# calad0i/da4ml

Hardware: AMD Instinct MI355X
Metric: CMVM solves/sec, 256x256 int8 matrix (higher is better)
Workload: dtype u32; 1 GPU; c3_256x256_int8_batch64_single_chain; matrix=256x256 int8 (default_rng(seed).integers(-128,128)), batch_per_gpu=64, parallelism=1 x independent-instance shard, no data-path collective

## Files before the change

da4ml_amd/csrc/cmvm_engine.hip:

```cpp

#include <hip/hip_runtime.h>

#include <algorithm>
#include <atomic>
#include <chrono>
#include <cmath>
#include <cstdio>
#include <cstdlib>
#include <cstring>
#include <memory>
#include <mutex>
#include <numeric>
#include <stdexcept>
#include <string>
#include <thread>
#include <type_traits>
#include <vector>

#include "cmvm_core.h"
#include "cmvm_geometry.h"
#include "cmvm_gpu.h"
#include "cmvm_host.h"

namespace da {
// ... 1383 lines not shown
            if constexpr (MANYCOL) {
                if (!same) rlB[pos - 1] = F::pack(colA, nbv);
            } else {
                if (!same) s_bent[pos - 1] = F::pack(colA, nbv);
            }
            rlN[at] = F::pack(colA, ma);
            mcol[at] = (int)colA;
            mA[at] = ma;
            mB[at] = mb;
            s_cm[colA] = (Idx)(at + 1);
            {
                DA_GLOBAL uint32_t *cb = colbits + (size_t)colA * cbw;
                atomicOr(gen(&cb[Nw >> 5]), 1u << (Nw & 31));
                if (na == 0) atomicAnd(gen(&cb[A >> 5]), ~(1u << (A & 31)));
                if (!same && nbv == 0) atomicAnd(gen(&cb[B >> 5]), ~(1u << (B & 31)));
            }
            if constexpr (MANYCOL)
                s_len[at] = collen[colA];
            else
                s_len[at] = s_clen[colA];
            s_col[at] = (Idx)colA;
            my_matches += popc32(O::plus(ma) | O::minus(ma));
        }
        if (na) for_pairs_self<Cell>(na, nb, [&](int k) { atomicAdd(&cAA[k], 1u); });
        if (!same) {
            if (na && nbv) for_pairs_cross<Cell>(na, nbv, nb, [&](int k) { atomicAdd(&cAB[k], 1u); });
            if (nbv && ma) for_pairs_cross<Cell>(nbv, ma, nb, [&](int k) { atomicAdd(&cBN[k], 1u); });
        }
        if (na && ma) for_pairs_cross<Cell>(na, ma, nb, [&](int k) { atomicAdd(&cAN[k], 1u); });
        if (ma) for_pairs_self<Cell>(ma, nb, [&](int k) { atomicAdd(&cNN[k], 1u); });
        m += chunk;
        __syncthreads();
    }
    if (my_matches) atomicAdd(&s_matches, my_matches);
    if (!same)
        for (int t = tid; t < lenB; t += SEL2_THREADS) {
            Entry e;
            if constexpr (MANYCOL)
                e = rlB[t];
            else {
                e = s_bent[t];
                rlB[t] = e;
            }
            const Cell nbv = F::cell(e);
            if (nbv) for_pairs_self<Cell>(nbv, nb, [&](int k) { atomicAdd(&cBB[k], 1u); });
        }
    for (int j = tid; j < n_out; j += SEL2_THREADS) cmap[j] = (uint16_t)s_cm[j];
    {
        const unsigned long long refN = ref_pack(Nw, (uint32_t)m, offN);
        for (int k = tid; k < m; k += SEL2_THREADS) {
            const int j = s_col[k], len = s_len[k];
            if (len < lcap) {
                collist[(size_t)j * lcap + len] = refN;
                collen[j] = len + 1;
            } else
                g->error = E_LIST_CAPACITY;
        }
    }
    __syncthreads();
    SEL_TIMER_MARK(4)
    SEL_TIMER_MARK(5)
    if constexpr (SHARDED) {
        for (int k = tid; k < 6 * c.K; k += SEL2_THREADS) {
            const int sp = k / c.K;
            cs_slab[k] = (same && (sp == 1 || sp == 2 || sp == 4)) ? 0 : (int32_t)s_cnt[sp * Kpad + (k - sp * c.K)];
        }
    } else
        for (int k = tid; k < 6 * Kpad; k += SEL2_THREADS) sp_cnt[k] = s_cnt[k];
    {
        const DA_GLOBAL uint32_t *cb = colbits;
        const int nwords = (int)((Nw + 31) >> 5), chunks = (nwords + WAVE - 1) / WAVE;
        DA_GLOBAL uint32_t *ids = pl_ids;
        const bool split = chunks * 4 <= NW && m >= 8 && nwords <= claim_words;
        if (split) {
            const int c = wid % chunks, part = wid / chunks, ways = (NW - c + chunks - 1) / chunks;
            const int w = c * WAVE + lane;
            if (w < nwords) {
                uint32_t bits = 0;
                for (int k = part; k < m; k += ways) bits |= cb[(size_t)s_col[k] * cbw + w];
                if (bits) atomicOr(&s_or[w], bits);
            }
            __syncthreads();
        }
        for (int wb = wid * WAVE; wb < nwords; wb += SEL2_THREADS) {
            const int w = wb + lane;
            uint32_t bits = 0;
            if (w < nwords) {
                if (split)
                    bits = s_or[w];
                else
                    for (int k = 0; k < m; ++k) bits |= cb[(size_t)s_col[k] * cbw + w];
                if ((int)(A >> 5) == w) bits &= ~(1u << (A & 31));
                if ((int)(B >> 5) == w) bits &= ~(1u << (B & 31));
                if ((int)(Nw >> 5) == w) bits &= ~(1u << (Nw & 31));
            }
            if constexpr (SHARDED) {
                const int fw = (int)((Nw + 3) / 4);
                if (w < nwords) {
#pragma unroll
                    for (int q = 0; q < 8; ++q) {
                        const uint32_t b = (bits >> (4 * q)) & 0xFu;
                        if (8 * w + q < fw) cs_flags[8 * w + q] = (int32_t)((b & 1u) | ((b & 2u) << 7) | ((b & 4u) << 14) | ((b & 8u) << 21));
                    }
                }
                continue;
            }
            const int cnt = popc32(bits), inc = (int)wave_scan_add_u32((uint32_t)cnt);
            const int wave_total = __builtin_amdgcn_readlane(inc, WAVE - 1);
            if (wave_total == 0) continue;
            int base = 0;
            if (lane == 0) base = atomicAdd(&s_np, wave_total);
            int at = __builtin_amdgcn_readfirstlane(base) + inc - cnt;
            while (bits) {
                const uint32_t id = (uint32_t)(w << 5) + (uint32_t)ctz32(bits);
                if (at < IDS_LDS)
                    s_ids[at] = id;
                else
                    ids[at] = id;
                ++at;
                bits &= bits - 1;
            }
        }
    }
    SEL_TIMER_MARK(6)
    __syncthreads();
    if constexpr (SHARDED) {
        if (tid < SHARD_TRAILER) cs_flags[(int)((Nw + 3) / 4) + tid] = 0;
    }
    {
        const int np = s_np;
        const DA_GLOBAL uint32_t *ids = pl_ids;
        for (int t = tid; t < np; t += 2 * SEL2_THREADS) {
            const int t2 = t + SEL2_THREADS;
            const bool has2 = t2 < np;
            const uint32_t r1 = t < IDS_LDS ? s_ids[t] : ids[t];
            const uint32_t r2 = !has2 ? r1 : t2 < IDS_LDS ? s_ids[t2] : ids[t2];
            const da_u2 ro1 = rowoff[r1], ro2 = rowoff[r2];
            load_fence();
            plist[t] = ref_pack(r1, ro1.y, ro1.x);
            if (has2) plist[t2] = ref_pack(r2, ro2.y, ro2.x);
        }
    }
    SEL_TIMER_MARK(7)
    if (tid == 0) {
        SEL_TIMER_FLUSH
        rowoff[Nw] = da_u2{offN, (uint32_t)m};
        g->rl_used = offN + (uint32_t)m;
        g->m = m;
        g->n_partners = s_np;
        atomicAdd(&g->st_matches, (unsigned long long)s_matches);
        atomicAdd(&g->st_partners, (unsigned long long)s_np);
        atomicAdd(&g->st_cells, (unsigned long long)s_np * (unsigned)m);
        if (fast) atomicAdd(&g->st_fast, 1ull);
        {
            const unsigned long long eb = sizeof(Entry), cb = sizeof(Cell);
            const unsigned long long nwords = (Nw + 31) >> 5;
            atomicAdd(&g->st_sel_bytes, 4ull * (unsigned)n_out + 64ull + 2ull * eb * (unsigned)(lenA + (same ? 0 : lenB)) + 4ull * (unsigned)m * nwords + 20ull * (unsigned)s_np +
                                            (unsigned)m * (4ull + 2ull * cb + eb + 8ull + 12ull) + 2ull * (unsigned)n_out + 6ull * 4ull * (unsigned)Kpad);
        }
        g->A = A;
        g->B = B;
        g->Nw = Nw;
        g->pk_shift = shift;
        g->pk_sub = sub;
        g->n_rows = (int)Nw + 1;
        g->iter = iter + 1;
    }
    return 0;
}
#ifndef DA_SEL2_WAVES
#define DA_SEL2_WAVES 4
#endif
template <class Cell, bool SHARDED = false, bool MANYCOL = false, bool SEEDED = false> __global__ void __launch_bounds__(SEL2_THREADS) __attribute__((amdgpu_waves_per_eu(DA_SEL2_WAVES, DA_SEL2_WAVES))) k_iter_select2(ChainDev *chains, int n_chains, unsigned int *n_done, int step) {
    if ((int)blockIdx.x >= n_chains) return;
#ifdef DA_STEP_CLOCKS
    {
        ChainDev *g = &chains[blockIdx.x];
        if (threadIdx.x == 0 && !g->done) {
            CLK_MARK(g, step & 1, 0, true);
            if (blockIdx.y == 1 && step > 0) {
                unsigned long long *k = g->clk[(step - 1) & 1];
                if (k[0] && k[1] && k[2] && k[3] && CLK_TIMED_STEP(step - 1)) {
                    g->st_qdiag[0] += k[1] - ~k[0];
                    g->st_qdiag[1] += ~k[2] - k[1];
                    g->st_qdiag[4] += k[3] - ~k[2];
                    g->st_qdiag[5] += CLK_NOW() - k[3];
                    g->st_qdiag[7] += 1;
                }
                k[0] = k[1] = k[2] = k[3] = 0;
            }
        }
    }
#endif
    if (blockIdx.y == 0)
        search_body<Cell, SEEDED>(&chains[blockIdx.x], step);
    else
        (void)pick_body<Cell, SHARDED, MANYCOL, SEEDED>(&chains[blockIdx.x], n_done, step);
#ifdef DA_STEP_CLOCKS
    __syncthreads();
    if (threadIdx.x == 0) CLK_MARK(&chains[blockIdx.x], step & 1, 1, false);
#endif
}

#ifndef DA_UPD_OCC
#define DA_UPD_OCC 5
#endif
#if DA_UPD_OCC >= 8
#define DA_UPD_SGPRS 80
#elif DA_UPD_OCC == 7
#define DA_UPD_SGPRS 96
#else
#define DA_UPD_SGPRS 102
#endif
constexpr int SLOT_NONE = -1, SLOT_SLOW = -2;

#ifndef DA_UPD_QG
#define DA_UPD_QG 16
#endif
constexpr int QG = DA_UPD_QG, QN = WAVE / QG;
constexpr int QG_LOG2 = QG == 16 ? 4 : 3, SPL = (int)BUCKET / QG, HL = QG / 2;
constexpr uint32_t QMASK = (1u << QG) - 1u, HMASK = (1u << HL) - 1u;
static_assert(QG == 16 || QG == 8, "a partner row is handled by one DPP row or half a row");

__device__ __forceinline__ unsigned long long row_max_u64(unsigned long long v) {
    v = dpp_max_u64<DPP_ROW_SHR1, 0xF>(v);
    v = dpp_max_u64<DPP_ROW_SHR2, 0xF>(v);
    v = dpp_max_u64<DPP_ROW_SHR4, 0xF>(v);
    v = dpp_max_u64<DPP_ROW_SHR8, 0xF>(v);
    return v;
}

constexpr int DPP_QUAD_XOR1 = 0xB1, DPP_QUAD_XOR2 = 0x4E, DPP_ROW_HALF_MIRROR = 0x141;
template <int LANES> __device__ __forceinline__ unsigned long long part_row_max_u64(unsigned long long v) {
    v = dpp_max_u64<DPP_QUAD_XOR1, 0xF>(v);
    v = dpp_max_u64<DPP_QUAD_XOR2, 0xF>(v);
    if constexpr (LANES == 8) v = dpp_max_u64<DPP_ROW_HALF_MIRROR, 0xF>(v);
    return v;
}

template <class Cell> struct UpdStep {
    Ctx c;
    int done, n_partners, m, n_in;
    uint32_t A, B, Nw;
    int shift, sub;
    const DA_GLOBAL int *mcol;
    const DA_GLOBAL Cell *mA, *mB;
    const DA_GLOBAL uint16_t *cmap;
    const DA_GLOBAL typename RowFmt<Cell>::Entry *rl;
    const DA_GLOBAL unsigned long long *plist;
    uint32_t dcw;
};
template <class Cell, bool SEEDED = false, bool WEIGHTED = false> __device__ __forceinline__ UpdStep<Cell> load_upd_step(ChainDev *gq) {
    using Entry = typename RowFmt<Cell>::Entry;
    UpdStep<Cell> u;
    int iter = gq->iter;
    u.done = gq->done, u.n_partners = gq->n_partners, u.m = gq->m, u.n_in = gq->n_in;
    u.A = gq->A, u.B = gq->B, u.Nw = gq->Nw;
    u.shift = gq->pk_shift, u.sub = gq->pk_sub;
    u.c = make_ctx_raw<SEEDED>(gq, 2 * iter - 1);
    if constexpr (WEIGHTED)
        u.dcw = f2u(gq->dc_weight);
    else
        u.dcw = 0;
    u.c.rword = gq->spec[(iter - 1) & 1].word;
    u.c.cn = &gq->c_n[(iter - 1) & 1];
    u.c.cl = &gq->c_list[(iter - 1) & 1][0];
    u.mcol = (const DA_GLOBAL int *)gq->mcol;
    u.mA = (const DA_GLOBAL Cell *)gq->mA, u.mB = (const DA_GLOBAL Cell *)gq->mB;
    u.cmap = (const DA_GLOBAL uint16_t *)gq->cmap;
    u.rl = (const DA_GLOBAL Entry *)gq->rlist;
    u.plist = (const DA_GLOBAL unsigned long long *)gq->plist;
    pin_sgpr(u.done, u.n_partners, iter, u.m, u.n_in, u.A, u.B, u.Nw, u.shift, u.sub, u.mcol, u.mA, u.cmap, u.rl, u.plist);
    pin_sgpr(u.c.n_out, u.c.n_bits, u.c.K, u.c.Kpad, u.c.method, u.c.gs_log2, u.c.pb_log2, u.c.cmask, u.c.windows, u.c.hkey, u.c.hrank, u.c.hblk, u.c.grec, u.c.rows);
    pin_sgpr(u.c.rword, u.c.cn, u.c.cl);
    if constexpr (SEEDED) pin_sgpr(u.c.seed);
    if constexpr (WEIGHTED) pin_sgpr(u.dcw);
    u.c.tomb = KEY_TOMB - (unsigned long long)((2 * iter - 1) & 3);
    ctx_finish(u.c);
    return u;
}
template <class Cell> struct UpdLds {
    Cell *mA, *mB;
    int *col;
    uint16_t *cmap;
    uint32_t *cnt;
    static __device__ __forceinline__ size_t table_bytes(int n_out) { return (size_t)n_out * (2 * sizeof(Cell) + 4 + 2); }
    static __device__ __forceinline__ size_t wave_bytes(int Kpad) { return (size_t)(QN * 3 + 1) * Kpad * 4; }
    __device__ __forceinline__ void carve(unsigned char *tables, unsigned char *counters, int n_out) {
        mA = reinterpret_cast<Cell *>(tables);
        mB = mA + n_out;
        col = reinterpret_cast<int *>(mB + n_out);
        cmap = reinterpret_cast<uint16_t *>(col + n_out);
        cnt = reinterpret_cast<uint32_t *>(counters);
    }
};
template <class Cell> __device__ __forceinline__ void copy_handoff(const UpdStep<Cell> &u, const UpdLds<Cell> &s, int t, int nthr) {
    for (int j = t; j < u.c.n_out; j += nthr) s.cmap[j] = u.cmap[j];
    for (int j = t; j < u.m; j += nthr) {
        s.col[j] = u.mcol[j];
        s.mA[j] = u.mA[j];
    }
}

template <class Cell, bool STATS, bool SEEDED = false, bool WEIGHTED = false>
__device__ __forceinline__ void update_partners(ChainDev *g, const UpdStep<Cell> &u, const UpdLds<Cell> &s, int first, int stride, int limit, unsigned long long ref_next,
                                                const RowInfo &rnew, unsigned int &found, unsigned int &inserts, unsigned int &deletes) {
    using F = RowFmt<Cell>;
    using Entry = typename F::Entry;
    constexpr int HW = ((sizeof(Cell) == 4 ? 24 : 60) + HL - 1) / HL;
    const Ctx &c = u.c;
    const uint32_t dcw = u.dcw;
    const uint32_t A = u.A, B = u.B, Nw = u.Nw;
    const int m = u.m, n_in = u.n_in, pk_shift = u.shift, pk_sub = u.sub;
    const DA_GLOBAL Entry *rl = u.rl;
    const DA_GLOBAL unsigned long long *plist = u.plist;
    Cell *s_mA = s.mA;
    int *s_col = s.col;
    uint16_t *s_cmap = s.cmap;
    uint32_t *s_cnt = s.cnt;
    const int nb = c.n_bits, Kpad = c.Kpad, K = c.K;
    const int lane = lane_id();
    const int q = lane >> QG_LOG2, l = lane & (QG - 1), qsh = q * QG;
    const bool same = A == B;
    uint32_t *dA = s_cnt + (size_t)q * 3 * Kpad, *dB = dA + Kpad, *cN = dB + Kpad;
    const int KW = Kpad / 2;
    UPD_TIMER_DECL
#ifndef DA_UPD_CH
#define DA_UPD_CH 4
#endif
    constexpr int CH = DA_UPD_CH;
    for (int base = first; base < limit; base += stride) {
        const int idx = base + q;
        const bool valid = idx < limit;
        const unsigned long long ref = ref_next;
        ref_next = idx + stride < limit ? plist[idx + stride] : 0ull;
        const uint32_t pr = ref_row(ref), off = ref_off(ref);
        const bool dense = valid && (int)pr < n_in;
        const int cnt = !valid ? 0 : dense ? m : (int)ref_len(ref);
        const uint32_t lA = min(A, pr), hA = max(A, pr), lB = min(B, pr), hB = max(B, pr);
        const unsigned long long keyA = pack_pair(lA, hA), keyB = pack_pair(lB, hB);
        const uint32_t baseA = (hash_pair(lA, hA) & ~(BUCKET - 1)) & c.cmask, baseB = (hash_pair(lB, hB) & ~(BUCKET - 1)) & c.cmask;
        unsigned long long kA[SPL], kB[SPL];
#pragma unroll
        for (int t = 0; t < SPL; ++t) {
            kA[t] = valid ? c.hkey[baseA + l * SPL + t] : KEY_TOMB;
            kB[t] = (valid && !same) ? c.hkey[baseB + l * SPL + t] : KEY_TOMB;
        }
        Entry e[CH];
#pragma unroll
        for (int u = 0; u < CH; ++u) {
            const int j = l + u * QG;
            e[u] = j < cnt ? rl[(size_t)off + (dense ? s_col[j] : j)] : F::none();
        }
        for (int k = l; k < 3 * Kpad; k += QG) dA[k] = 0;
        int sA = SLOT_NONE, sB = SLOT_NONE;
        {
            bool emp_a = false, emp_b = false;
            int at_a = -1, at_b = -1;
#pragma unroll
            for (int t = 0; t < SPL; ++t) {
                at_a = kA[t] == keyA ? t : at_a;
                at_b = kB[t] == keyB ? t : at_b;
                emp_a |= kA[t] == KEY_EMPTY;
                emp_b |= kB[t] == KEY_EMPTY;
            }
            const uint32_t hitA = (uint32_t)(__ballot(at_a >= 0) >> qsh) & QMASK, empA = (uint32_t)(__ballot(emp_a) >> qsh) & QMASK;
            const uint32_t hitB = (uint32_t)(__ballot(at_b >= 0) >> qsh) & QMASK, empB = (uint32_t)(__ballot(emp_b) >> qsh) & QMASK;
            int ta = 0, tb = 0;
            if constexpr (SPL > 1) {
                ta = __shfl(at_a, hitA ? qsh + ctz32(hitA) : lane);
                tb = __shfl(at_b, hitB ? qsh + ctz32(hitB) : lane);
            }
            if (valid) {
                sA = hitA ? (int)(baseA + (uint32_t)(ctz32(hitA) * SPL + ta)) : (empA ? SLOT_NONE : SLOT_SLOW);
                if (!same) sB = hitB ? (int)(baseB + (uint32_t)(ctz32(hitB) * SPL + tb)) : (empB ? SLOT_NONE : SLOT_SLOW);
            }
        }
        UPD_TIMER_MARK(1)
        const int half = l / HL, hl = l % HL;
        const int sX = half ? sB : sA;
        const unsigned long long keyX = half ? keyB : keyA;
        const da_i4 z4 = da_i4{0, 0, 0, 0};
        const da_i4 hdX = sX >= 0 ? *reinterpret_cast<const DA_GLOBAL da_i4 *>(blk_ptr(c, sX)) : z4;
        uint32_t wX[HW];
#pragma unroll
        for (int u = 0; u < HW; ++u) {
            const int j = hl + u * HL;
            wX[u] = (sX >= 0 && j < KW) ? reinterpret_cast<const DA_GLOBAL uint32_t *>(blk_ptr(c, sX) + 16)[j] : 0u;
        }
        lds_fence();
        const bool hasA = sA != SLOT_NONE, hasB = same ? hasA : sB != SLOT_NONE;
        const bool mirA = A < pr, mirB = same ? mirA : B < pr;
        const int Wk4 = 4 * (2 * nb - 1), sgnA4 = mirA ? -4 : 4, sgnB4 = mirB ? -4 : 4, tau = pk_sub ? -1 : 1;
        unsigned char *const spare = reinterpret_cast<unsigned char *>(s_cnt + (size_t)QN * 3 * Kpad);
        unsigned char *const pN = reinterpret_cast<unsigned char *>(cN + (nb - 1));
        unsigned char *const pA = (hasA ? reinterpret_cast<unsigned char *>(dA) : spare) + 4 * (nb - 1);
        unsigned char *const pB = (hasB ? reinterpret_cast<unsigned char *>(same ? dA : dB) : spare) + 4 * (nb - 1) + (pk_sub ? Wk4 : 0) + sgnB4 * pk_shift;
        auto bump = [](unsigned char *at) { atomicAdd(reinterpret_cast<uint32_t *>(at), 1u); };
        auto pairs_of = [&](const Entry en) {
            using O = CellOps<Cell>;
            const Cell x = F::cell(en);
            const int at = x ? (int)s_cmap[F::col(en)] : 0;
            if (!at) return;
            const Cell ma = s_mA[at - 1];
            const uint32_t xm = O::minus(x), hm = O::minus(ma), la0 = O::plus(x) | xm;
            uint32_t h = O::plus(ma) | hm;
            while (h) {
                const int q_ = ctz32(h);
                h &= h - 1;
                const uint32_t xq = (hm >> q_) & 1u ? ~xm : xm;
                uint32_t la = la0;
                while (la) {
                    const int p_ = ctz32(la);
                    la &= la - 1;
                    int sgm = -(int)((xq >> p_) & 1u);
                    pin_vgpr(sgm);
                    const int d = q_ - p_, off = sgm & Wk4;
                    bump(pN + off + 4 * d);
                    bump(pA + off + __mul24(d, sgnA4));
                    bump(pB + __mul24(off, tau) + __mul24(d, sgnB4));
                }
            }
        };
#pragma unroll
        for (int u = 0; u < CH; ++u)
            if (__any(u * QG < cnt)) pairs_of(e[u]);
        for (int j = l + CH * QG; __any(j < cnt); j += QG)
            if (j < cnt) pairs_of(rl[(size_t)off + (dense ? s_col[j] : j)]);
        lds_fence();
        int fnew = 0;
        for (int k = l; k < K; k += QG) fnew |= cN[k] >= 2u;
        const bool gnew = valid && (((uint32_t)(__ballot(fnew != 0) >> qsh) & QMASK) != 0);
        UPD_TIMER_MARK(2)
        {
            const bool has = sX >= 0;
            const int ov = hdX.x;
            const float dl = __int_as_float(hdX.y);
            const uint32_t *d = half ? dB : dA;
            unsigned long long best = 0;
            int alive = 0;
#pragma unroll
            for (int u = 0; u < HW; ++u) {
                const int j = hl + u * HL;
                if (has && j < KW) {
                    const uint32_t o0 = wX[u] & 0xFFFFu, o1 = wX[u] >> 16;
                    const uint32_t n0 = o0 - d[2 * j], n1 = o1 - d[2 * j + 1];
                    if (n0 != o0 || n1 != o1) reinterpret_cast<DA_GLOBAL uint32_t *>(blk_ptr(c, sX) + 16)[j] = (n0 & 0xFFFFu) | (n1 << 16);
                    alive |= (n0 >= 2u) | (n1 >= 2u);
                    const uint32_t r0 = rank_of<WEIGHTED>(c, dcw, n0, ov, dl), r1 = rank_of<WEIGHTED>(c, dcw, n1, ov, dl);
                    const unsigned long long c0 = r0 ? (((unsigned long long)r0 << 8) | blk_pos<SEEDED>((unsigned)(2 * j), c.seed)) : 0ull;
                    const unsigned long long c1 = r1 ? (((unsigned long long)r1 << 8) | blk_pos<SEEDED>((unsigned)(2 * j + 1), c.seed)) : 0ull;
                    best = c0 > best ? c0 : best;
                    best = c1 > best ? c1 : best;
                }
            }
            best = part_row_max_u64<HL>(best);
            const bool any_alive = (((uint32_t)(__ballot(alive != 0) >> (qsh + HL * half)) & HMASK) != 0);
            if (has && hl == HL - 1) block_commit<SEEDED>(c, sX, keyX, BlkHdr{ov, dl, (uint32_t)hdX.z, (uint32_t)hdX.w}, best, any_alive, false);
            if constexpr (STATS) deletes += (unsigned)__popcll(__ballot(has && hl == HL - 1 && !any_alive));
        }
        UPD_TIMER_MARK(3)
        bool gslow = false;
        if (__ballot(gnew)) {
            const unsigned long long keyN = pack_pair(pr, Nw);
            const uint32_t baseN = (hash_pair(pr, Nw) & ~(BUCKET - 1)) & c.cmask;
            unsigned long long kN[SPL];
#pragma unroll
            for (int t = 0; t < SPL; ++t) kN[t] = gnew ? c.hkey[baseN + l * SPL + t] : 0ull;
            const RowInfo rp = load_row(c.rows, gnew ? pr : 0u);
            int pick_t = -1;
#pragma unroll
            for (int t = SPL - 1; t >= 0; --t)
                if (gnew && (kN[t] == KEY_EMPTY || (kN[t] >= KEY_TOMB_LO && kN[t] != c.tomb))) pick_t = t;
            uint32_t av = (uint32_t)(__ballot(pick_t >= 0) >> qsh) & QMASK;
            int nslot = -1;
            bool trying = gnew;
            while (__ballot(trying)) {
                const int cand = av ? ctz32(av) : -1;
                int ok = 0;
                if (trying && l == cand) {
                    const unsigned long long was = pick_t == 0 ? kN[0] : kN[SPL - 1];
                    ok = atomicCAS(gen(&c.hkey[baseN + l * SPL + pick_t]), was, keyN) == was;
                }
                const bool won = (((uint32_t)(__ballot(ok != 0) >> qsh)) & QMASK) != 0;
                int tsel = 0;
                if constexpr (SPL > 1) tsel = __shfl(pick_t, cand >= 0 ? qsh + cand : lane);
                if (trying) {
                    if (cand < 0) {
                        trying = false;
                        gslow = true;
                    } else if (won) {
                        nslot = (int)(baseN + (uint32_t)(cand * SPL + tsel));
                        trying = false;
                    } else
                        av &= av - 1;
                }
            }
            const bool made = nslot >= 0;
            const int ovn = n_overlap(rp, rnew);
            const float dln = fabsf(rp.lat - rnew.lat);
            unsigned long long bestn = 0;
            constexpr int CWN = ((sizeof(Cell) == 4 ? 24 : 60) + QG - 1) / QG;
#pragma unroll
            for (int u = 0; u < CWN; ++u) {
                const int j = l + u * QG;
                if (made && j < KW) {
                    const uint32_t n0 = cN[2 * j], n1 = cN[2 * j + 1];
                    if ((n0 | n1) > 65535u) c.g->error = E_COUNT_OVERFLOW;
                    reinterpret_cast<DA_GLOBAL uint32_t *>(blk_ptr(c, nslot) + 16)[j] = (n0 & 0xFFFFu) | (n1 << 16);
                    const uint32_t r0 = rank_of<WEIGHTED>(c, dcw, n0, ovn, dln), r1 = rank_of<WEIGHTED>(c, dcw, n1, ovn, dln);
                    const unsigned long long c0 = r0 ? (((unsigned long long)r0 << 8) | blk_pos<SEEDED>((unsigned)(2 * j), c.seed)) : 0ull;
                    const unsigned long long c1 = r1 ? (((unsigned long long)r1 << 8) | blk_pos<SEEDED>((unsigned)(2 * j + 1), c.seed)) : 0ull;
                    bestn = c0 > bestn ? c0 : bestn;
                    bestn = c1 > bestn ? c1 : bestn;
                }
            }
            bestn = part_row_max_u64<8>(bestn);
            if constexpr (QG == 16) bestn = dpp_max_u64<0x140, 0xF>(bestn);
            if (made && l == QG - 1) {
                const uint32_t rank = (uint32_t)(bestn >> 8), bidx = blk_pos<SEEDED>((uint32_t)(bestn & 0xFF), c.seed);
                store_hdr(c, nslot, ovn, dln, rank, bidx);
                c.hrank[nslot] = rank;
                hidx_ptr(c)[nslot] = (uint8_t)bidx;
                if (rank) {
                    group_note(c, nslot, 0ull, bound_word(rank, tie_of<SEEDED>(pr, Nw, (int)bidx, c.seed)));
                    fold_entry(c, rank, tie_of<SEEDED>(pr, Nw, (int)bidx, c.seed));
                }
            }
            if constexpr (STATS) inserts += (unsigned)__popcll(__ballot(made && l == 0));
        }
        const unsigned long long rare = __ballot(valid && (sA == SLOT_SLOW || sB == SLOT_SLOW || gslow));
        if constexpr (STATS) found += (unsigned)__popcll(__ballot(l == 0 && sA >= 0)) + (unsigned)__popcll(__ballot(l == 0 && sB >= 0));
        if (rare) {
#pragma unroll 1
            for (int qq = 0; qq < QN; ++qq) {
                if (!((rare >> (qq * QG)) & 1ull)) continue;
                const uint32_t rpr = (uint32_t)__builtin_amdgcn_readlane((int)pr, qq * QG);
                const int rsA = __builtin_amdgcn_readlane(sA, qq * QG), rsB = __builtin_amdgcn_readlane(sB, qq * QG);
                const int rnewb = __builtin_amdgcn_readlane((int)gslow, qq * QG);
                const uint32_t *rdA = s_cnt + (size_t)qq * 3 * Kpad, *rdB = rdA + Kpad, *rcN = rdB + Kpad;
                if (rsA == SLOT_SLOW) {
                    const uint32_t lo = min(A, rpr), hi = max(A, rpr);
                    const int slot = table_find_from(c, pack_pair(lo, hi), hash_pair(lo, hi), 1);
                    if (slot >= 0) {
                        int gone = 0;
                        table_update<SEEDED, WEIGHTED>(c, slot, pack_pair(lo, hi), [&](int k, uint32_t old) { return old - rdA[k]; }, false, &gone, dcw);
                        if constexpr (STATS) deletes += (unsigned)gone, ++found;
                    }
                }
                if (rsB == SLOT_SLOW) {
                    const uint32_t lo = min(B, rpr), hi = max(B, rpr);
                    const int slot = table_find_from(c, pack_pair(lo, hi), hash_pair(lo, hi), 1);
                    if (slot >= 0) {
                        int gone = 0;
                        table_update<SEEDED, WEIGHTED>(c, slot, pack_pair(lo, hi), [&](int k, uint32_t old) { return old - rdB[k]; }, false, &gone, dcw);
                        if constexpr (STATS) deletes += (unsigned)gone, ++found;
                    }
                }
                if (rnewb) {
                    table_insert<SEEDED, WEIGHTED>(c, rpr, Nw, load_row(c.rows, rpr), rnew, [&](int k) { return rcN[k]; }, nullptr, false, dcw);
                    if constexpr (STATS) ++inserts;
                }
            }
        }
        UPD_TIMER_PASS_END
        lds_fence();
    }
    UPD_TIMER_FLUSH
}

template <class Cell, bool SEEDED = false, bool WEIGHTED = false> __device__ __forceinline__ void special_pairs(ChainDev *gq, const UpdStep<Cell> &u, int part) {
    const Ctx &c = u.c;
    const uint32_t A = u.A, B = u.B, Nw = u.Nw;
    const bool same = A == B;
    const DA_GLOBAL uint32_t *spc = (const DA_GLOBAL uint32_t *)gq->sp_cnt;
    const RowInfo ra = load_row(c.rows, A), rb = load_row(c.rows, B), rn = load_row(c.rows, Nw);
    const int lane = lane_id();
    for (int sp = part * UPD_WAVES + wave_id(); sp < min(6, (part + 1) * UPD_WAVES); sp += UPD_WAVES) {
        uint32_t lo = A, hi = A;
        bool active = true, existed = false;
        int row = 0;
        switch (sp) {
        case 0: lo = A, hi = A, existed = true, row = 0; break;
        case 1: lo = A, hi = B, existed = true, active = !same, row = 1; break;
        case 2: lo = A, hi = Nw, row = 3; break;
        case 3: lo = B, hi = B, existed = true, active = !same, row = 2; break;
        case 4: lo = B, hi = Nw, active = !same, row = 4; break;
        default: lo = Nw, hi = Nw, row = 5; break;
        }
        if (!active) continue;
        const DA_GLOBAL uint32_t *cnt = spc + (size_t)row * c.Kpad;
        const unsigned long long key = pack_pair(lo, hi);
        const int slot = existed ? table_find(c, key, hash_pair(lo, hi)) : -1;
        unsigned long long w = 0;
        if (slot >= 0)
            w = table_update<SEEDED, WEIGHTED>(c, slot, key, [&](int k, uint32_t) { return cnt[k]; }, true, nullptr, u.dcw);
        else {
            int f = 0;
            for (int k = lane; k < c.K; k += WAVE) f |= cnt[k] >= 2u;
            if (__any(f)) {
                const RowInfo xa = pick_row(lo == Nw, rn, pick_row(lo == A, ra, rb)), xb = pick_row(hi == Nw, rn, pick_row(hi == A, ra, rb));
                table_insert<SEEDED, WEIGHTED>(c, lo, hi, xa, xb, [&](int k) { return cnt[k]; }, &w, true, u.dcw);
            }
        }
        (void)w;
    }
    if (c.rword && part == 1) {
        const int nl = (int)gq->l_n[(gq->iter - 1) & 1];
        const CandEntry *ll = &gq->l_list[(gq->iter - 1) & 1][0];
        const uint32_t *colbits = gq->colbits;
        const int cbw = gq->cb_words;
        for (int e = (wave_id() + 2) % UPD_WAVES; e < nl; e += UPD_WAVES) {
            const unsigned long long tw = ll[e].tie;
            uint32_t i0, i1;
            tie_rows<SEEDED>(tw, c.seed, i0, i1);
            const uint32_t r = (i0 == A || i0 == B) ? i1 : i0;
            int hit = 0;
            for (int k = lane; k < u.m; k += WAVE) hit |= (int)((colbits[(size_t)u.mcol[k] * cbw + (r >> 5)] >> (r & 31)) & 1u);
            if (!__any(hit) && lane == 0) fold_entry(c, (uint32_t)ll[e].rank, tw);
        }
    }
}

template <class Cell, int NWV, bool STATS, bool SEEDED = false, bool WEIGHTED = false>
__device__ __forceinline__ void update_body(ChainDev *gq, bool in_range, int block_y, int grid_y) {
    constexpr int NTHR = NWV * WAVE;
    const UpdStep<Cell> u = load_upd_step<Cell, SEEDED, WEIGHTED>(gq);
    if (!in_range || u.done) return;
    if (block_y >= grid_y - 2) {
        special_pairs<Cell, SEEDED, WEIGHTED>(gq, u, block_y - (grid_y - 2));
        return;
    }
    grid_y -= 2;
    if (block_y * (NWV * QN) >= u.n_partners) return;
    extern __shared__ __attribute__((aligned(16))) unsigned char smem[];
    const int tid = threadIdx.x, lane = lane_id(), wid = wave_id();
    UpdLds<Cell> s;
    s.carve(smem, smem + align16(UpdLds<Cell>::table_bytes(u.c.n_out)) + (size_t)wid * UpdLds<Cell>::wave_bytes(u.c.Kpad), u.c.n_out);
    const int total_waves = grid_y * NWV, gw = block_y * NWV + wid;
    const unsigned long long ref0 = gw * QN + (lane >> QG_LOG2) < u.n_partners ? u.plist[gw * QN + (lane >> QG_LOG2)] : 0ull;
    const RowInfo rnew = load_row(u.c.rows, u.Nw);
    __shared__ unsigned int s_stat[3];
    if constexpr (STATS)
        if (tid < 3) s_stat[tid] = 0;
    copy_handoff<Cell>(u, s, tid, NTHR);
    __syncthreads();
    unsigned int found = 0, inserts = 0, deletes = 0;
    update_partners<Cell, STATS, SEEDED, WEIGHTED>(gq, u, s, gw * QN, total_waves * QN, u.n_partners, ref0, rnew, found, inserts, deletes);
    if constexpr (!STATS) return;
    if (lane == 0 && (found | inserts | deletes)) {
        if (found) atomicAdd(&s_stat[0], found);
        if (inserts) atomicAdd(&s_stat[1], inserts);
        if (deletes) atomicAdd(&s_stat[2], deletes);
    }
    __syncthreads();
    if (tid == 0) {
        if (s_stat[0]) atomicAdd(&gq->st_found, (unsigned long long)s_stat[0]);
        if (s_stat[1]) atomicAdd(&gq->st_inserts, (unsigned long long)s_stat[1]);
        if (s_stat[1] != s_stat[2]) atomicAdd(&gq->n_live, s_stat[1] - s_stat[2]);
    }
}
template <class Cell, bool STATS, bool SEEDED = false, bool WEIGHTED = false>
__global__ void __launch_bounds__(UPD_THREADS, DA_UPD_OCC) __attribute__((amdgpu_num_sgpr(DA_UPD_SGPRS))) k_iter_update(ChainDev *chains, int n_chains) {
#ifdef DA_STEP_CLOCKS
    ChainDev *gk = &chains[(int)blockIdx.x < n_chains ? blockIdx.x : 0];
    const bool clk_on = (int)blockIdx.x < n_chains && !gk->done;
    const int clk_par = (gk->iter - 1) & 1;
    if (clk_on && threadIdx.x == 0) CLK_MARK(gk, clk_par, 2, true);
#endif
    update_body<Cell, UPD_WAVES, STATS, SEEDED, WEIGHTED>(&chains[(int)blockIdx.x < n_chains ? blockIdx.x : 0], (int)blockIdx.x < n_chains, (int)blockIdx.y, (int)gridDim.y);
#ifdef DA_STEP_CLOCKS
    __syncthreads();
    if (clk_on && threadIdx.x == 0) CLK_MARK(gk, clk_par, 3, false);
#endif
}


template <class Cell> __global__ void __launch_bounds__(256) k_cs_init_counts(ChainDev *g) {
    const Ctx c = make_ctx(g, 0);
    extern __shared__ __attribute__((aligned(16))) unsigned char smem[];
    uint32_t *cnt = reinterpret_cast<uint32_t *>(smem) + (size_t)wave_id() * c.Kpad;
    const long long n_in = g->n_in, n_pairs = n_in * (n_in + 1) / 2;
    const long long p = (long long)blockIdx.x * (blockDim.x / WAVE) + wave_id();
    if (p >= n_pairs) return;
    long long i1 = (long long)((sqrt(8.0 * (double)p + 1.0) - 1.0) * 0.5);
    while (i1 * (i1 + 1) / 2 > p) --i1;
    while ((i1 + 1) * (i1 + 2) / 2 <= p) ++i1;
    const uint32_t hi = (uint32_t)i1, lo = (uint32_t)(p - i1 * (i1 + 1) / 2);
    count_row_pair<Cell>(c, reinterpret_cast<const typename RowFmt<Cell>::Entry *>(g->rlist), lo, hi, cnt);
    for (int k = lane_id(); k < c.K; k += WAVE) g->cs_init[(size_t)p * c.K + k] = (int32_t)cnt[k];
}
template <class Cell> __global__ void __launch_bounds__(256) k_cs_init_table(ChainDev *g) {
    const Ctx c = make_ctx(g, 0);
    const long long n_in = g->n_in, n_pairs = n_in * (n_in + 1) / 2;
    const long long p = (long long)blockIdx.x * (blockDim.x / WAVE) + wave_id();
    if (p >= n_pairs) return;
    long long i1 = (long long)((sqrt(8.0 * (double)p + 1.0) - 1.0) * 0.5);
    while (i1 * (i1 + 1) / 2 > p) --i1;
    while ((i1 + 1) * (i1 + 2) / 2 <= p) ++i1;
    const uint32_t hi = (uint32_t)i1, lo = (uint32_t)(p - i1 * (i1 + 1) / 2);
    const int32_t *cnt = g->cs_init + (size_t)p * c.K;
    int f = 0;
    for (int k = lane_id(); k < c.K; k += WAVE) f |= cnt[k] >= 2;
    if (!__any(f)) return;
    if (c.method < 0) {
        if (lane_id() == 0) g->unknown_hit = 1;
        return;
    }
    table_insert(c, lo, hi, load_row(c.rows, lo), load_row(c.rows, hi), [&](int k) { return (uint32_t)cnt[k]; });
}

__global__ void __launch_bounds__(1024) k_cs_union(ChainDev *g, volatile int *report, int seq, int flag_words) {
    __shared__ int s_part[16], s_base[17];
    const int tid = threadIdx.x, lane = lane_id(), wid = wave_id();
    const int n_rows = (int)g->Nw;
    const int per = (n_rows + 1023) / 1024;
    const int r0 = min(tid * per, n_rows), r1 = min(r0 + per, n_rows);
    int mine = 0;
    for (int r = r0; r < r1; ++r) mine += ((g->cs_flags[r >> 2] >> (8 * (r & 3))) & 0xFF) != 0;
    int inc = mine;
    for (int o = 1; o < WAVE; o <<= 1) {
        int t = __shfl_up(inc, o);
        if (lane >= o) inc += t;
    }
    if (lane == WAVE - 1) s_part[wid] = inc;
    __syncthreads();
    if (tid == 0) {
        int run = 0;
        for (int w = 0; w < 16; ++w) {
            s_base[w] = run;
            run += s_part[w];
        }
        s_base[16] = run;
        g->cs_nuni = run;
        if (report) {
            report[1] = run;
            report[2] = g->cs_flags[flag_words];
            report[3] = g->cs_flags[flag_words + 1];
            report[4] = g->cs_flags[flag_words + 2];
            __threadfence_system();
            report[0] = seq;
        }
    }
    __syncthreads();
    int at = s_base[wid] + inc - mine;
    for (int r = r0; r < r1; ++r)
        if (((g->cs_flags[r >> 2] >> (8 * (r & 3))) & 0xFF) != 0) g->cs_uni[at++] = (uint32_t)r;
}

template <class Cell> __global__ void __launch_bounds__(256) k_cs_partial(ChainDev *g) {
    using F = RowFmt<Cell>;
    using Entry = typename F::Entry;
    const Ctx c = make_ctx(g, 0);
    const int m = g->m, nb = c.n_bits, n_out = c.n_out, K = c.K, Kpad = c.Kpad;
    extern __shared__ __attribute__((aligned(16))) unsigned char smem[];
    Cell *s_mA = reinterpret_cast<Cell *>(smem);
    Cell *s_mB = s_mA + n_out;
    uint32_t *s_cnt = reinterpret_cast<uint32_t *>(s_mB + n_out);
    uint16_t *s_cmap = reinterpret_cast<uint16_t *>(s_cnt + 4 * 3 * Kpad);
    const int tid = threadIdx.x, lane = lane_id(), wid = wave_id();
    for (int j = tid; j < n_out; j += 256) s_cmap[j] = 0;
    __syncthreads();
    for (int j = tid; j < m; j += 256) {
        s_cmap[g->mcol[j]] = (uint16_t)(j + 1);
        s_mA[j] = reinterpret_cast<const Cell *>(g->mA)[j];
        s_mB[j] = reinterpret_cast<const Cell *>(g->mB)[j];
    }
    __syncthreads();
    const int u = (int)blockIdx.x * 4 + wid;
    if (u >= g->cs_nuni) return;
    const uint32_t A = g->A, B = g->B, r = g->cs_uni[u];
    const bool same = A == B;
    uint32_t *dA = s_cnt + (size_t)wid * 3 * Kpad, *dB = dA + Kpad, *cN = dB + Kpad;
    for (int k = lane; k < 3 * Kpad; k += WAVE) dA[k] = 0;
    lds_fence();
    const da_u2 ref = g->rowoff[r];
    const Entry *row = reinterpret_cast<const Entry *>(g->rlist) + ref.x;
    for (int j = lane; j < (int)ref.y; j += WAVE) {
        const Entry en = row[j];
        const Cell x = F::cell(en);
        if (!x) continue;
        const int at = (int)s_cmap[F::col(en)];
        if (!at) continue;
        const Cell ma = s_mA[at - 1], mb = s_mB[at - 1];
        for_pairs_part<Cell>(ma, x, A < r, nb, [&](int k) { atomicAdd(&dA[k], 1u); });
        if (same)
            for_pairs_part<Cell>(mb, x, A < r, nb, [&](int k) { atomicAdd(&dA[k], 1u); });
        else
            for_pairs_part<Cell>(mb, x, B < r, nb, [&](int k) { atomicAdd(&dB[k], 1u); });
        for_pairs_cross<Cell>(x, ma, nb, [&](int k) { atomicAdd(&cN[k], 1u); });
    }
    lds_fence();
    int32_t *out = g->cs_slab + (size_t)(6 + 3 * u) * K;
    for (int k = lane; k < K; k += WAVE) {
        out[k] = (int32_t)dA[k];
        out[K + k] = (int32_t)dB[k];
        out[2 * K + k] = (int32_t)cN[k];
    }
}

template <class Cell> __global__ void __launch_bounds__(256) k_cs_apply(ChainDev *g) {
    Ctx c = make_ctx(g, 2 * g->iter - 1);
    c.rword = g->spec[(g->iter - 1) & 1].word;
    c.cn = &g->c_n[(g->iter - 1) & 1];
    c.cl = &g->c_list[(g->iter - 1) & 1][0];
    const int K = c.K;
    const int w = (int)blockIdx.x * 4 + wave_id();
    const uint32_t A = g->A, B = g->B, Nw = g->Nw;
    const bool same = A == B;
    if (w == 5 && c.rword) {
        const int nl = (int)g->l_n[(g->iter - 1) & 1];
        const CandEntry *ll = &g->l_list[(g->iter - 1) & 1][0];
        if (lane_id() == 0)
            for (int e = 0; e < nl; ++e) {
                const unsigned long long tw = ll[e].tie;
                const uint32_t i0 = (uint32_t)((tw >> 7) & 0xFFFFFFu), i1 = (uint32_t)(tw >> 31);
                const uint32_t r = (i0 == A || i0 == B) ? i1 : i0;
                if (((g->cs_flags[r >> 2] >> (8 * (r & 3))) & 0xFF) == 0) fold_entry(c, (uint32_t)ll[e].rank, tw);
            }
    }
    if (w < 6) {
        uint32_t lo = A, hi = A;
        bool active = true, existed = false;
        switch (w) {
        case 0: lo = A, hi = A, existed = true; break;
        case 1: lo = A, hi = B, existed = true, active = !same; break;
        case 2: lo = B, hi = B, existed = true, active = !same; break;
        case 3: lo = A, hi = Nw; break;
        case 4: lo = B, hi = Nw, active = !same; break;
        default: lo = Nw, hi = Nw; break;
        }
        if (!active) return;
        const int32_t *cnt = g->cs_slab + (size_t)w * K;
        const unsigned long long key = pack_pair(lo, hi);
        const int slot = existed ? table_find(c, key, hash_pair(lo, hi)) : -1;
        if (slot >= 0)
            table_update(c, slot, key, [&](int k, uint32_t) { return (uint32_t)cnt[k]; });
        else {
            int f = 0;
            for (int k = lane_id(); k < K; k += WAVE) f |= cnt[k] >= 2;
            if (__any(f)) table_insert(c, lo, hi, load_row(c.rows, lo), load_row(c.rows, hi), [&](int k) { return (uint32_t)cnt[k]; });
        }
        return;
    }
    const int u = w - 6;
    if (u >= g->cs_nuni) return;
    const uint32_t r = g->cs_uni[u];
    const int32_t *dA = g->cs_slab + (size_t)(6 + 3 * u) * K, *dB = dA + K, *cN = dB + K;
    {
        const uint32_t lo = min(A, r), hi = max(A, r);
        const int slot = table_find(c, pack_pair(lo, hi), hash_pair(lo, hi));
        if (slot >= 0) table_update(c, slot, pack_pair(lo, hi), [&](int k, uint32_t old) { return old - (uint32_t)dA[k]; });
    }
    if (!same) {
        const uint32_t lo = min(B, r), hi = max(B, r);
        const int slot = table_find(c, pack_pair(lo, hi), hash_pair(lo, hi));
        if (slot >= 0) table_update(c, slot, pack_pair(lo, hi), [&](int k, uint32_t old) { return old - (uint32_t)dB[k]; });
    }
// ... 157 lines not shown
```

Before: 112.1 solves/s.

## Derive partner loss counts from single new-pair histogram instead of three atomic histograms

The inner pair loop used to do three LDS atomic increments per digit pair, one each into the new-pair, A-loss and B-loss histograms. It now bumps only the new-pair histogram. The A and B decrement vectors are rebuilt on the fly by index remapping (sign mirroring, shift and subtract-offset) through a helper, which cuts LDS atomics and LDS footprint to a third. In exchange, each consumer does extra index arithmetic and conditional LDS reads, and the lane id is re-pinned in VGPRs to control register pressure. Correctness depends on the remapping exactly matching the former offset formulas, including the same-row case.

Result: no change. 113.7 solves/s, median of 6 (+1.5%).

```diff
diff --git a/da4ml_amd/csrc/cmvm_engine.hip b/da4ml_amd/csrc/cmvm_engine.hip
--- a/da4ml_amd/csrc/cmvm_engine.hip
+++ b/da4ml_amd/csrc/cmvm_engine.hip
@@ -1709,6 +1709,11 @@
     }
 }
 
+__device__ __forceinline__ uint32_t upd_loss(const uint32_t *cN, int k, int K, int W, int nbm1, int sgn, int cst, int sub) {
+    const int sg = k >= W, t = __mul24(k - (sg ? W : 0) - nbm1, sgn) + cst;
+    return (k < K && (unsigned)t < (unsigned)W) ? cN[((sg ^ sub) ? W : 0) + t] : 0u;
+}
+
 template <class Cell, bool STATS, bool SEEDED = false, bool WEIGHTED = false>
 __device__ __forceinline__ void update_partners(ChainDev *g, const UpdStep<Cell> &u, const UpdLds<Cell> &s, int first, int stride, int limit, unsigned long long ref_next,
                                                 const RowInfo &rnew, unsigned int &found, unsigned int &inserts, unsigned int &deletes) {
@@ -1727,9 +1732,13 @@
     uint32_t *s_cnt = s.cnt;
     const int nb = c.n_bits, Kpad = c.Kpad, K = c.K;
     const int lane = lane_id();
-    const int q = lane >> QG_LOG2, l = lane & (QG - 1), qsh = q * QG;
+    auto lane_now = [&]() {
+        int v = lane;
+        pin_vgpr(v);
+        return v;
+    };
     const bool same = A == B;
-    uint32_t *dA = s_cnt + (size_t)q * 3 * Kpad, *dB = dA + Kpad, *cN = dB + Kpad;
+    const int W = 2 * nb - 1;
     const int KW = Kpad / 2;
     UPD_TIMER_DECL
 #ifndef DA_UPD_CH
@@ -1737,6 +1746,8 @@
 #endif
     constexpr int CH = DA_UPD_CH;
     for (int base = first; base < limit; base += stride) {
+        const int ln = lane_now(), q = ln >> QG_LOG2, l = ln & (QG - 1), qsh = q * QG;
+        uint32_t *const cN = s_cnt + (size_t)q * Kpad;
         const int idx = base + q;
         const bool valid = idx < limit;
         const unsigned long long ref = ref_next;
@@ -1759,7 +1770,7 @@
             const int j = l + u * QG;
             e[u] = j < cnt ? rl[(size_t)off + (dense ? s_col[j] : j)] : F::none();
         }
-        for (int k = l; k < 3 * Kpad; k += QG) dA[k] = 0;
+        for (int k = l; k < Kpad; k += QG) cN[k] = 0;
         int sA = SLOT_NONE, sB = SLOT_NONE;
         {
             bool emp_a = false, emp_b = false;
@@ -1786,7 +1797,6 @@
         UPD_TIMER_MARK(1)
         const int half = l / HL, hl = l % HL;
         const int sX = half ? sB : sA;
-        const unsigned long long keyX = half ? keyB : keyA;
         const da_i4 z4 = da_i4{0, 0, 0, 0};
         const da_i4 hdX = sX >= 0 ? *reinterpret_cast<const DA_GLOBAL da_i4 *>(blk_ptr(c, sX)) : z4;
         uint32_t wX[HW];
@@ -1796,13 +1806,8 @@
             wX[u] = (sX >= 0 && j < KW) ? reinterpret_cast<const DA_GLOBAL uint32_t *>(blk_ptr(c, sX) + 16)[j] : 0u;
         }
         lds_fence();
-        const bool hasA = sA != SLOT_NONE, hasB = same ? hasA : sB != SLOT_NONE;
-        const bool mirA = A < pr, mirB = same ? mirA : B < pr;
-        const int Wk4 = 4 * (2 * nb - 1), sgnA4 = mirA ? -4 : 4, sgnB4 = mirB ? -4 : 4, tau = pk_sub ? -1 : 1;
-        unsigned char *const spare = reinterpret_cast<unsigned char *>(s_cnt + (size_t)QN * 3 * Kpad);
+        const int Wk4 = 4 * W;
         unsigned char *const pN = reinterpret_cast<unsigned char *>(cN + (nb - 1));
-        unsigned char *const pA = (hasA ? reinterpret_cast<unsigned char *>(dA) : spare) + 4 * (nb - 1);
-        unsigned char *const pB = (hasB ? reinterpret_cast<unsigned char *>(same ? dA : dB) : spare) + 4 * (nb - 1) + (pk_sub ? Wk4 : 0) + sgnB4 * pk_shift;
         auto bump = [](unsigned char *at) { atomicAdd(reinterpret_cast<uint32_t *>(at), 1u); };
         auto pairs_of = [&](const Entry en) {
             using O = CellOps<Cell>;
@@ -1824,8 +1829,6 @@
                     pin_vgpr(sgm);
                     const int d = q_ - p_, off = sgm & Wk4;
                     bump(pN + off + 4 * d);
-                    bump(pA + off + __mul24(d, sgnA4));
-                    bump(pB + __mul24(off, tau) + __mul24(d, sgnB4));
                 }
             }
         };
@@ -1840,10 +1843,18 @@
         const bool gnew = valid && (((uint32_t)(__ballot(fnew != 0) >> qsh) & QMASK) != 0);
         UPD_TIMER_MARK(2)
         {
+            const int ln = lane_now(), q = ln >> QG_LOG2, l = ln & (QG - 1), qsh = q * QG, half = l / HL, hl = l % HL;
+            const uint32_t *const cN = s_cnt + (size_t)q * Kpad;
             const bool has = sX >= 0;
             const int ov = hdX.x;
             const float dl = __int_as_float(hdX.y);
-            const uint32_t *d = half ? dB : dA;
+            const uint32_t rowX = half ? B : A;
+            const int sgnX = rowX < pr ? -1 : 1, cstX = half ? nb - 1 - pk_shift : nb - 1, subX = half ? pk_sub : 0;
+            auto lost = [&](int k) {
+                uint32_t v = upd_loss(cN, k, K, W, nb - 1, sgnX, cstX, subX);
+                if (same) v += upd_loss(cN, k, K, W, nb - 1, sgnX, nb - 1 - pk_shift, pk_sub);
+                return v;
+            };
             unsigned long long best = 0;
             int alive = 0;
 #pragma unroll
@@ -1851,7 +1862,7 @@
                 const int j = hl + u * HL;
                 if (has && j < KW) {
                     const uint32_t o0 = wX[u] & 0xFFFFu, o1 = wX[u] >> 16;
-                    const uint32_t n0 = o0 - d[2 * j], n1 = o1 - d[2 * j + 1];
+                    const uint32_t n0 = o0 - lost(2 * j), n1 = o1 - lost(2 * j + 1);
                     if (n0 != o0 || n1 != o1) reinterpret_cast<DA_GLOBAL uint32_t *>(blk_ptr(c, sX) + 16)[j] = (n0 & 0xFFFFu) | (n1 << 16);
                     alive |= (n0 >= 2u) | (n1 >= 2u);
                     const uint32_t r0 = rank_of<WEIGHTED>(c, dcw, n0, ov, dl), r1 = rank_of<WEIGHTED>(c, dcw, n1, ov, dl);
@@ -1863,12 +1874,14 @@
             }
             best = part_row_max_u64<HL>(best);
             const bool any_alive = (((uint32_t)(__ballot(alive != 0) >> (qsh + HL * half)) & HMASK) != 0);
-            if (has && hl == HL - 1) block_commit<SEEDED>(c, sX, keyX, BlkHdr{ov, dl, (uint32_t)hdX.z, (uint32_t)hdX.w}, best, any_alive, false);
+            if (has && hl == HL - 1) block_commit<SEEDED>(c, sX, pack_pair(min(rowX, pr), max(rowX, pr)), BlkHdr{ov, dl, (uint32_t)hdX.z, (uint32_t)hdX.w}, best, any_alive, false);
             if constexpr (STATS) deletes += (unsigned)__popcll(__ballot(has && hl == HL - 1 && !any_alive));
         }
         UPD_TIMER_MARK(3)
         bool gslow = false;
         if (__ballot(gnew)) {
+            const int ln = lane_now(), q = ln >> QG_LOG2, l = ln & (QG - 1), qsh = q * QG;
+            const uint32_t *const cN = s_cnt + (size_t)q * Kpad;
             const unsigned long long keyN = pack_pair(pr, Nw);
             const uint32_t baseN = (hash_pair(pr, Nw) & ~(BUCKET - 1)) & c.cmask;
             unsigned long long kN[SPL];
@@ -1945,13 +1958,16 @@
                 const uint32_t rpr = (uint32_t)__builtin_amdgcn_readlane((int)pr, qq * QG);
                 const int rsA = __builtin_amdgcn_readlane(sA, qq * QG), rsB = __builtin_amdgcn_readlane(sB, qq * QG);
                 const int rnewb = __builtin_amdgcn_readlane((int)gslow, qq * QG);
-                const uint32_t *rdA = s_cnt + (size_t)qq * 3 * Kpad, *rdB = rdA + Kpad, *rcN = rdB + Kpad;
+                const uint32_t *rcN = s_cnt + (size_t)qq * Kpad;
+                const int rsgA = A < rpr ? -1 : 1, rsgB = B < rpr ? -1 : 1;
+                auto rdA = [&](int k) { return upd_loss(rcN, k, K, W, nb - 1, rsgA, nb - 1, 0) + (same ? upd_loss(rcN, k, K, W, nb - 1, rsgA, nb - 1 - pk_shift, pk_sub) : 0u); };
+                auto rdB = [&](int k) { return upd_loss(rcN, k, K, W, nb - 1, rsgB, nb - 1 - pk_shift, pk_sub); };
                 if (rsA == SLOT_SLOW) {
                     const uint32_t lo = min(A, rpr), hi = max(A, rpr);
                     const int slot = table_find_from(c, pack_pair(lo, hi), hash_pair(lo, hi), 1);
                     if (slot >= 0) {
                         int gone = 0;
-                        table_update<SEEDED, WEIGHTED>(c, slot, pack_pair(lo, hi), [&](int k, uint32_t old) { return old - rdA[k]; }, false, &gone, dcw);
+                        table_update<SEEDED, WEIGHTED>(c, slot, pack_pair(lo, hi), [&](int k, uint32_t old) { return old - rdA(k); }, false, &gone, dcw);
                         if constexpr (STATS) deletes += (unsigned)gone, ++found;
                     }
                 }
@@ -1960,7 +1976,7 @@
                     const int slot = table_find_from(c, pack_pair(lo, hi), hash_pair(lo, hi), 1);
                     if (slot >= 0) {
                         int gone = 0;
-                        table_update<SEEDED, WEIGHTED>(c, slot, pack_pair(lo, hi), [&](int k, uint32_t old) { return old - rdB[k]; }, false, &gone, dcw);
+                        table_update<SEEDED, WEIGHTED>(c, slot, pack_pair(lo, hi), [&](int k, uint32_t old) { return old - rdB(k); }, false, &gone, dcw);
                         if constexpr (STATS) deletes += (unsigned)gone, ++found;
                     }
                 }
```
